# facebookresearch/FRL-Distributed-ML-Scaffold

Measured on NVIDIA H100. Metric: samples/sec (whole box) on synthetic 2-task Problem, higher is better.
Workload: dtype bf16

## Files before the change

### frl-distributed-ml-scaffold_b200/_native.py

```python
import ctypes as C
import os
import subprocess
from typing import Optional, Sequence

import torch

_HERE = os.path.dirname(os.path.abspath(__file__))
CSRC_DIR = os.path.join(_HERE, "csrc")
LIB_PATH = os.path.join(CSRC_DIR, "libfrl_b200.so")

F32, BF16, U8, I64 = 0, 1, 2, 3
LOSS_MSE, LOSS_CE, LOSS_CE_PROB = 0, 1, 2
FP8_E4M3, FP8_E5M2 = 0, 1
FP8_DTYPE = {FP8_E4M3: torch.float8_e4m3fn, FP8_E5M2: torch.float8_e5m2}
MAX_TASKS = 8

_DTYPE_CODE = {torch.float32: F32, torch.bfloat16: BF16, torch.uint8: U8, torch.bool: U8,
               torch.int64: I64}


class NativeLibraryError(RuntimeError):
    pass


# ... 3 lines not shown
        ("ignore_index", C.c_int32),
        ("out", C.c_void_p), ("tgt", C.c_void_p), ("mask", C.c_void_p), ("dout", C.c_void_p),
        ("rows", C.c_int64), ("cols", C.c_int64), ("mask_inner", C.c_int64),
        ("weight", C.c_float), ("label_smoothing", C.c_float),
    ]


class GradSeg(C.Structure):
    _fields_ = [("g", C.c_void_p), ("arena_off", C.c_int64), ("numel", C.c_int64),
                ("g_dtype", C.c_int32), ("_pad", C.c_int32)]


_vp, _i, _i64, _f, _d = C.c_void_p, C.c_int, C.c_int64, C.c_float, C.c_double
SIGNATURES = {
    "frl_abi_version": (_i, []),
    "frl_last_error": (C.c_char_p, []),
    "frl_launch_count": (C.c_uint64, []),
    "frl_launch_count_reset": (None, []),
    "frl_device_sm_count": (_i, []),
    "frl_device_arch": (_i, []),
    "frl_sgd_momentum": (_i, [_vp, _vp, _vp, _vp, _i64, _d, _d, _d, _d, _d, _vp, _vp, _i, _i, _vp]),
    "frl_adam": (_i, [_vp, _vp, _vp, _vp, _vp, _vp, _i64, _d, _d, _d, _d, _d, _i64, _d, _vp, _vp, _i, _vp]),
    "frl_rmsprop": (_i, [_vp, _vp, _vp, _vp, _vp, _i64, _d, _d, _d, _d, _d, _d, _vp, _vp, _i, _vp]),
    "frl_mt_tile_elems": (_i64, []),
    "frl_flatten_grads": (_i, [_vp, _vp, _vp, _i64, _vp, _i, _d, _vp]),
    "frl_sgd_momentum_mt": (_i, [_vp, _vp, _vp, _vp, _vp, _vp, _i64, _d, _d, _d, _d, _d, _vp, _vp, _i, _vp]),
    "frl_adam_mt": (_i, [_vp, _vp, _vp, _vp, _vp, _vp, _vp, _vp, _i64, _d, _d, _d, _d, _d, _i64, _d, _vp, _vp, _vp]),
    "frl_rmsprop_mt": (_i, [_vp, _vp, _vp, _vp, _vp, _vp, _vp, _i64, _d, _d, _d, _d, _d, _d, _vp, _vp, _vp]),
    "frl_layerwise_scratch_bytes": (_i64, [_i64, _i64]),
    "frl_lars_mt": (_i, [_vp, _vp, _vp, _vp, _vp, _vp, _i64, _i64, _vp, _vp, _vp, _d, _d, _d, _d, _vp, _vp, _i, _vp]),
    "frl_lamb_mt": (_i, [_vp, _vp, _vp, _vp, _vp, _vp, _vp, _i64, _i64, _vp, _vp, _vp, _d, _d, _d, _d, _d, _i64,
                         _d, _vp, _vp, _vp]),
    "frl_grad_accumulate_mt": (_i, [_vp, _vp, _vp, _vp, _i64, _d, _i, _vp, _vp]),
    "frl_weight_ema": (_i, [_vp, _vp, _i64, _d, _vp]),
    "frl_reduce_scratch_bytes": (_i64, []),
    "frl_grad_sumsq_clip": (_i, [_vp, _i64, _i, _f, _f, _vp, _vp, _vp]),
    "frl_criteria_scratch_bytes": (_i64, [_i]),
    "frl_criteria_forward": (_i, [C.POINTER(TaskDesc), _i, _vp, _vp, _vp, _vp, _vp, _vp, _vp]),
    "frl_criteria_backward": (_i, [C.POINTER(TaskDesc), _i, _vp, _vp, _vp, _vp]),
    "frl_preproc_affine": (_i, [_vp, _i, _vp, _i, _i64, _i64, _i64, _vp, _vp, _vp]),
    "frl_cast_scale": (_i, [_vp, _i, _vp, _i, _i64, _f, _vp]),
    "frl_augment_images": (_i, [_vp, _i64, _i, _i, _i, _vp, C.c_uint64, _i, _i, _d, _d, _d, _d, _d, _i, _i,
                                _vp, _vp, _vp, _i, _i, _i, _vp, _vp]),
    "frl_augment_mix_images": (_i, [_vp, _i64, _i, _i, _i, _vp, C.c_uint64, _i, _i, _d, _d, _d, _d, _d, _i, _i,
                                    _vp, _vp, _vp, _i, _i, _i, _vp, _i, _f, _i, _i, _i, _i, _vp]),
    "frl_mix_targets": (_i, [_vp, _i, _i64, _i64, _i, _f, _vp, _vp]),
# ... 89 lines not shown

def sgd_momentum(p, g, buf, p_lp, n, *, lr, mu, dampening, wd, grad_scale=1.0,
                 grad_scale_dev=None, first_step=False, dyn=None) -> None:
    _check(lib().frl_sgd_momentum(_ptr(p), _ptr(g), _ptr(buf), _ptr(p_lp), n, lr, mu, dampening,
                                  wd, grad_scale, _ptr(grad_scale_dev), _ptr(dyn), int(first_step),
                                  dtype_code(g.dtype), _stream()), "frl_sgd_momentum")


def adam(p, g, m, v, vmax, p_lp, n, *, lr, beta1, beta2, eps, wd, step, grad_scale=1.0,
         grad_scale_dev=None, dyn=None) -> None:
    _check(lib().frl_adam(_ptr(p), _ptr(g), _ptr(m), _ptr(v), _ptr(vmax), _ptr(p_lp), n, lr,
                          beta1, beta2, eps, wd, step, grad_scale, _ptr(grad_scale_dev), _ptr(dyn),
                          dtype_code(g.dtype), _stream()), "frl_adam")


def rmsprop(p, g, sq, buf, p_lp, n, *, lr, alpha, eps, wd, mu, grad_scale=1.0,
            grad_scale_dev=None, dyn=None) -> None:
    _check(lib().frl_rmsprop(_ptr(p), _ptr(g), _ptr(sq), _ptr(buf), _ptr(p_lp), n, lr, alpha,
                             eps, wd, mu, grad_scale, _ptr(grad_scale_dev), _ptr(dyn),
                             dtype_code(g.dtype), _stream()), "frl_rmsprop")



def mt_tile_elems() -> int:
    return int(lib().frl_mt_tile_elems())


def flatten_grads(table, arena_grad, *, scale: float = 1.0) -> None:
    _check(lib().frl_flatten_grads(table.segs_dev_ptr, table.prefix_dev_ptr, table.tile_seg_dev_ptr, table.n_tiles,
                                   _ptr(arena_grad), dtype_code(arena_grad.dtype), scale, _stream()),
           "frl_flatten_grads")


def sgd_momentum_mt(p, buf, p_lp, table, *, lr, mu, dampening, wd, grad_scale=1.0, grad_scale_dev=None,
                    first_step=False, dyn=None) -> None:
    _check(lib().frl_sgd_momentum_mt(_ptr(p), _ptr(buf), _ptr(p_lp), table.segs_dev_ptr, table.prefix_dev_ptr,
                                     table.tile_seg_dev_ptr, table.n_tiles, lr, mu, dampening, wd, grad_scale,
                                     _ptr(grad_scale_dev), _ptr(dyn), int(first_step), _stream()),
           "frl_sgd_momentum_mt")


def adam_mt(p, m, v, vmax, p_lp, table, *, lr, beta1, beta2, eps, wd, step, grad_scale=1.0,
            grad_scale_dev=None, dyn=None) -> None:
    _check(lib().frl_adam_mt(_ptr(p), _ptr(m), _ptr(v), _ptr(vmax), _ptr(p_lp), table.segs_dev_ptr,
                             table.prefix_dev_ptr, table.tile_seg_dev_ptr, table.n_tiles, lr, beta1, beta2, eps, wd,
                             step, grad_scale, _ptr(grad_scale_dev), _ptr(dyn), _stream()), "frl_adam_mt")
# ... 342 lines not shown
```

### frl-distributed-ml-scaffold_b200/arena_linear.py

```python
import os
import types
from collections import Counter
from typing import List, Optional

import torch
import torch.nn as nn
import torch.nn.functional as F

from . import _native
from .types import Precision

KERNELS = _native

FP8_MULTIPLE = 16


def fp8_site_qualifies(uses_lp: bool, in_features: int, out_features: int) -> bool:
    return bool(uses_lp) and in_features % FP8_MULTIPLE == 0 and out_features % FP8_MULTIPLE == 0


def fp8_call_qualifies(x: torch.Tensor) -> bool:
    if x.dim() == 0 or x.shape[-1] == 0 or x.dtype not in (torch.bfloat16, torch.float32):
        return False
    m = x.numel() // x.shape[-1]
# ... 255 lines not shown

class LinearSite:
    __slots__ = ("module", "wslot", "bslot", "pipeline", "relu", "wstate", "bstate", "multihead", "fp8")

    def __init__(self, module, wslot, bslot, pipeline):
        self.module = module
        self.wslot = wslot
        self.bslot = bslot
        self.pipeline = pipeline
        self.relu = None
        self.multihead = None
        self.fp8 = False
        states = pipeline.slot_states
        self.wstate = states.setdefault(wslot.index, SlotState())
        self.bstate = states.setdefault(bslot.index, SlotState()) if bslot is not None else None

    def weight_grad(self, pipe, gemms) -> None:
        gw = pipe.arena.grad_view(self.wslot)
        st = self.wstate
        if not st.first_touch(pipe.step_id):
            gemms.dw_add(gw)
            return
        rows = pipe.row_split(self.wslot)
        if (rows and rows % gemms.row_multiple == 0 and st.fwd_gen == pipe.forward_gen
                and st.fwd_count == 1):
            gemms.dw(gemms.dzt[:rows], out=gw[:rows])
            pipe.rows_ready(self.wslot, rows)
            gemms.dw(gemms.dzt[rows:], out=gw[rows:])
        else:
            gemms.dw(gemms.dzt, out=gw)

    def count_forward(self) -> None:
        pipe = self.pipeline
        if pipe is not None and self.module.training and torch.is_grad_enabled():
            gen = pipe.forward_gen
            self.wstate.count_forward(gen)
            if self.bstate is not None:
                self.bstate.count_forward(gen)

    def backward_done(self, pipe) -> None:
        step, gen = pipe.step_id, pipe.forward_gen
        if self.wstate.backward_complete(step, gen):
            pipe.mark_ready(self.wslot)
        else:
            pipe.defer_ready(self.wslot)
        if self.bstate is not None:
            if self.bstate.backward_complete(step, gen):
                pipe.mark_ready(self.bslot)
            else:
                pipe.defer_ready(self.bslot)

# ... 114 lines not shown
```

### frl-distributed-ml-scaffold_b200/fused_optim.py

```python
from typing import Any, Dict, List, Optional, Tuple

import torch

from . import _native
from .arena import ParamArena
from .types import LayerAdaptation, OptAlgorithm, OptimOpts

KERNELS = _native


class FusedArenaOptimizer(torch.optim.Optimizer):

    STATE_NAMES: Tuple[str, ...] = ()

    @property
    def needs_whole_tensors(self) -> bool:
        return False

    def __init__(self, arena: ParamArena, defaults: Dict[str, Any]) -> None:
        self.arena = arena
        params = arena.all_params
        if not params:
            raise ValueError("optimizer got an empty parameter list")
        super().__init__(params, defaults)
# ... 167 lines not shown
            elif entry:
                steps = max(steps, 1)
        self._steps = steps


class FusedSGD(FusedArenaOptimizer):
    STATE_NAMES = (("momentum_buffer", "momentum_buffer"),)

    def __init__(self, arena, lr, momentum=0.0, dampening=0.0, weight_decay=0.0):
        super().__init__(arena, dict(lr=lr, momentum=momentum, dampening=dampening,
                                     weight_decay=weight_decay, nesterov=False, maximize=False,
                                     foreach=None, differentiable=False, fused=None))

    def _launch(self, lo, hi, grad_scale, coef):
        h = self.hyper
        p, g, lp = self._slices(lo, hi)
        mu = float(h["momentum"])
        buf = self._state("momentum_buffer")[lo:hi] if mu != 0.0 else None
        KERNELS.sgd_momentum(p, g, buf, lp, hi - lo, lr=float(h["lr"]), mu=mu,
                             dampening=float(h["dampening"]), wd=float(h["weight_decay"]),
                             grad_scale=grad_scale, grad_scale_dev=coef,
                             first_step=(self._steps == 0), dyn=self._dyn)

    def _launch_mt(self, table, grad_scale):
        h = self.hyper
        mu = float(h["momentum"])
        KERNELS.sgd_momentum_mt(self.arena.master, self._state("momentum_buffer") if mu != 0.0 else None,
                                self.arena.lp, table, lr=float(h["lr"]), mu=mu,
                                dampening=float(h["dampening"]), wd=float(h["weight_decay"]),
                                grad_scale=grad_scale, first_step=(self._steps == 0), dyn=self._dyn)

    def _launch_nvls(self, lo, hi, grad_scale):
        h = self.hyper
        mu = float(h["momentum"])
        mc_g, mc_out = self._nvls_ptrs(lo)
        buf = self._state("momentum_buffer")[lo:hi] if mu != 0.0 else None
        KERNELS.nvls_sgd(self.arena.master[lo:hi], buf, mc_g, mc_out, hi - lo, self.nvls,
                         lr=float(h["lr"]), mu=mu, dampening=float(h["dampening"]),
                         wd=float(h["weight_decay"]), grad_scale=grad_scale,
                         first_step=(self._steps == 0),
                         g_dtype=KERNELS.dtype_code(self.arena.grad.dtype), dyn=self._dyn)


class FusedAdam(FusedArenaOptimizer):
    STATE_NAMES = (("exp_avg", "exp_avg"), ("exp_avg_sq", "exp_avg_sq"),
                   ("max_exp_avg_sq", "max_exp_avg_sq"))
# ... 214 lines not shown
```

### frl-distributed-ml-scaffold_b200/grad_sync.py

```python
import os
from typing import Callable, Dict, List, NamedTuple, Optional, Tuple

import torch
import torch.distributed as dist
import torch.nn as nn

from . import _native
from .arena import ParamArena
from .fused_optim import FusedArenaOptimizer

KERNELS = _native


class MicroBatch(NamedTuple):
    first: bool
    closes: bool
    rows: int
    weight: float
    group_rows: int


def accumulation_plan(n_batches: int, k: int, batch_size: int = 1,
                      n_samples: Optional[int] = None) -> List[MicroBatch]:
    if n_batches <= 0:
        return []
    last = batch_size if n_samples is None else n_samples - (n_batches - 1) * batch_size
    if not 0 < last <= batch_size:
        raise ValueError("%r samples do not make %d batches of %d" % (n_samples, n_batches, batch_size))
    rows = [batch_size] * (n_batches - 1) + [last]
    plan: List[MicroBatch] = []
    for lo in range(0, n_batches, k):
        group = rows[lo:lo + k]
# ... 119 lines not shown
        self._deferred = {}
        self.mt_enabled = (self.on_cuda and hasattr(KERNELS, "flatten_grads")
                           and os.environ.get("FRL_B200_MT_GRADS", "1") != "0")
        self._ext: Dict[int, torch.Tensor] = {}
        self.tables = _TableSet(arena)
        self._keep_ext = False
        self.record_update_events = False
        self.update_events: List[Tuple[torch.cuda.Event, torch.cuda.Event, int, int]] = []
        self.accumulate_events: List[Tuple[torch.cuda.Event, torch.cuda.Event]] = []

        self.acc: Optional[torch.Tensor] = None
        if self.accumulation > 1:
            self.acc = torch.zeros(arena.numel, dtype=torch.float32, device=arena.device)
            self._acc_dyn = torch.ones(2, dtype=torch.float32, device=arena.device)
            self._acc_dyn_host = torch.zeros(self._ACC_RING, 2, dtype=torch.float32, pin_memory=self.on_cuda)
            self._acc_dyn_slot = 0
            self._acc_dyn_last: Optional[Tuple[float, float]] = (1.0, 1.0)
        self._acc_first = True
        self._acc_closes = True
        self._acc_weight = 1.0
        self._acc_scale = self.grad_scale
        self._acc_seen = set()
        self.last_ready: frozenset = frozenset()

    _ACC_RING = 16

    @property
    def accumulator_bytes(self) -> int:
        return 0 if self.acc is None else self.acc.numel() * 4

    def set_microbatch(self, *, first: bool, closes: bool, weight: float = 1.0,
                       group_scale: float = 1.0) -> None:
        if self.acc is None:
            return
        self._acc_first, self._acc_closes = bool(first), bool(closes)
        self._acc_weight = float(weight)
        self._acc_scale = float(group_scale) / self.world
        if first:
            self._acc_seen.clear()
        vals = (self._acc_weight, 1.0 if first else 0.0)
        if vals != self._acc_dyn_last:
            if self.on_cuda:
                row = self._acc_dyn_host[self._acc_dyn_slot % self._ACC_RING]
                self._acc_dyn_slot += 1
                row[0], row[1] = vals
                self._acc_dyn.copy_(row, non_blocking=True)
            else:
                self._acc_dyn.copy_(torch.tensor(vals, dtype=torch.float32))
            self._acc_dyn_last = vals

    def begin_step(self) -> None:
        self._ready = 0
        self._ready_ids.clear()
        self._deferred.clear()
        for b in self.buckets:
            b.pending = len(b.slots)
            b.work = None
            b.launched = False
        self.optimizer.begin_step()
        self.step_id += 1
        self._step_open = True

    @property
    def step_open(self) -> bool:
        return self._step_open

    def _make_hook(self, slot) -> Callable[[nn.Parameter], None]:
        from .multi_tensor import grad_usable_in_place

        def hook(param: nn.Parameter) -> None:
            g = param.grad
            if g is not None:
                dst = self.arena.grad_view(slot)
                if g.data_ptr() != dst.data_ptr():
                    if self.mt_enabled and self._step_open and grad_usable_in_place(g, slot):
                        self._ext[slot.index] = g
                    else:
                        dst.copy_(g)
                param.grad = None
            self.mark_ready(slot)
        return hook

# ... 33 lines not shown
    def mark_ready(self, slot) -> None:
        if not self._step_open or id(slot.param) in self._ready_ids:
            return
        self._ready_ids.add(id(slot.param))
        self._ready += 1
        for b in self._buckets_of[id(slot.param)]:
            if b.launched:
                continue
            b.pending -= 1
            if b.pending == 0 and (self.distributed or self.eager) and self.acc is None:
                self._launch_bucket(b)

    def row_split(self, slot) -> int:
        return self._row_split.get(slot.index, 0)

    def rows_ready(self, slot, rows: int) -> None:
        if not self._step_open:
            return
        done = slot.offset + rows * slot.shape[1]
        for b in self._buckets_of[id(slot.param)]:
            if not b.launched and b.hi <= done and b.pending == 1:
                b.pending = 0
                self._launch_bucket(b)

    def defer_ready(self, slot) -> None:
        self._deferred[slot.index] = slot

    def _launch_bucket(self, b: _Bucket) -> None:
        if self.on_cuda:
            cur = torch.cuda.current_stream()
            self.side_stream.wait_stream(cur)
            torch.cuda.set_stream(self.side_stream)
        try:
            if self._ext:
                self._flatten_stragglers(b.slots, id(b), side=self.on_cuda)
            fused = self.nvls is not None and not b.replicated
            if self.distributed and not fused:
                b.work = dist.all_reduce(self.arena.grad[b.lo:b.hi], op=dist.ReduceOp.SUM,
                                         group=self.pg, async_op=True)
                if self.eager:
                    b.work.wait()
            if self.eager:
                tap = self._tap()
                if fused:
                    nv = self.nvls
                    grid = nv.max_blocks
# ... 42 lines not shown
            self._accumulate_microbatch(keep_refs=defer_tail)
        else:
            if self.distributed and not self.eager:
                cur = torch.cuda.current_stream() if self.on_cuda else None
                if cur is not None:
                    torch.cuda.set_stream(self.side_stream)
                for b in self.buckets:
                    b.work.wait()
                if cur is not None:
                    torch.cuda.set_stream(cur)
            if self.on_cuda and (self.distributed or self.eager):
                torch.cuda.current_stream().wait_stream(self.side_stream)
            if partial:
                self._end_update([s for s in self.arena.slots if id(s.param) in self._ready_ids],
                                 ema=not defer_tail)
                return
        if not defer_tail:
            self.run_tail()

    @property
    def has_tail(self) -> bool:
        return not self.eager

    def run_tail(self, grad_refs=None, tables=None, ready=None) -> None:
        if self.acc is not None:
            if ready is not None:
                self._acc_seen |= ready
            if self._acc_closes:
                self._end_update(acc=True)
            return
        if grad_refs is not None:
            mine = (self._ext, self.tables)
            self._ext, self.tables, self._keep_ext = grad_refs, tables, True
        try:
            if self.has_tail:
                self._end_update()
            else:
                self.optimizer.end_step()
                if self.ema is not None:
                    self.ema.update()
        finally:
            if grad_refs is not None:
                (self._ext, self.tables), self._keep_ext = mine, False

    def _end_update(self, present=None, acc: bool = False, ema: bool = True) -> None:
        slots, n = self.arena.slots, self.arena.numel
        if acc:
            grads, scale = self.acc, self._acc_scale
            if self.distributed:
                for b in self.buckets:
                    dist.all_reduce(grads[b.lo:b.hi], op=dist.ReduceOp.SUM, group=self.pg)
            else:
                present = [s for s in slots if s.index in self._acc_seen]
        else:
            grads, scale = self.arena.grad, self.grad_scale
        have = {s.index for s in (slots if present is None else present)}
        every = len(have) == len(slots)
        window = self._tap() if acc else None
        coef = None
        if not acc and (self.clip_norm > 0.0 or not every):
            self._flatten_stragglers(slots, "all", side=False)
        if self.clip_norm > 0.0:
            if not acc:
                for s in slots:
                    if s.index not in have and s.is_model:
                        grads[s.offset:s.end].zero_()
            n_model = self.arena.model_end
            KERNELS.grad_sumsq_clip(grads[:n_model], n_model, pre_scale=scale, max_norm=self.clip_norm,
                                    out3=self.clip_out, scratch=self.clip_scratch)
            coef = self.clip_out[2:3]
        if self.whole_tensors or (not acc and self._ext and coef is None and not self.distributed):
            table = self._table("acc" if acc else "grads", [s for s in slots if s.index in have], acc=acc)
            tap = None if acc else self._tap()
            self.optimizer.apply_table(table, grad_scale=scale, clip_coef_dev=coef)
            self._tap_end(tap, self.update_events, 0, n)
        else:
            done = [(b.lo, b.hi) for b in self.buckets if b.launched and self.eager]
            runs = [(0, n)] if every else self._runs(
                lambda s: s.index in have and not any(a <= s.offset < z for a, z in done))
            for lo, hi in runs:
                tap = None if acc else self._tap()
                self.optimizer.apply_range(lo, hi, grad_scale=scale, clip_coef_dev=coef,
                                           grad_src=grads if acc else None)
                self._tap_end(tap, self.update_events, lo, hi)
        self._tap_end(window, self.update_events, 0, n)
        if not self._keep_ext:
            self._ext.clear()
        self.optimizer.end_step()
        if ema and self.ema is not None:
            self.ema.update()

    def _runs(self, keep) -> List[Tuple[int, int]]:
        runs: List[Tuple[int, int]] = []
        run_lo = prev_end = None
        for s in self.arena.slots:
            if not keep(s):
                if run_lo is not None:
                    runs.append((run_lo, prev_end))
                    run_lo = None
                continue
            if run_lo is None:
# ... 92 lines not shown
```

### frl-distributed-ml-scaffold_b200/graph_step.py

```python
from typing import Dict, List, Optional, Sequence, Tuple

import gc
import logging

import torch

from . import _native

logger = logging.getLogger(__name__)

REPLAYED_LAUNCHES = 0


def _signature(data: Sequence[torch.Tensor], target) -> Tuple:
    sig = [(tuple(t.shape), t.dtype) for t in data]
    for head in target:
        sig.append(tuple((tuple(t.shape), t.dtype) for t in head))
    return tuple(sig)


class GraphedTrainStep:
    WARMUP_STEPS = 2

    def __init__(self, worker) -> None:
# ... 40 lines not shown
        for t in data:
            cast = bf16 and t.dtype == torch.float32
            self.static_in.append(torch.empty_like(t, dtype=torch.bfloat16 if cast else t.dtype))
            self.cast_in.append(cast)
        self.static_tgt = [tuple(torch.empty_like(t) for t in head) for head in target]
        self._fill(data, target)

        w.optimizer.enable_dynamic_scalars()
        w.criterion.set_step_sink(None, None)
        gc.collect()
        torch.cuda.synchronize()
        self.graph = torch.cuda.CUDAGraph()
        launches_before = _native.launch_count()
        with torch.cuda.graph(self.graph, capture_error_mode="thread_local"):
            if w.buffers is not None:
                w.buffers.sync()
            output = w.model(self.static_in)
            total, sub = w.criterion(output, self.static_tgt)
            w.pipeline.begin_step()
            total.backward()
            w.pipeline.finish_step(defer_tail=True)
        self.grad_refs, self.tables = w.pipeline.detach_grad_refs()
        self.ready = w.pipeline.last_ready
        w.pipeline.step_id -= 1
        self.frl_kernels = _native.launch_count() - launches_before
        self.output = [o.detach() for o in output]
        self.names = list(sub.keys())
        self._total, self._sub = total.detach(), {k: v.detach() for k, v in sub.items()}
        base = getattr(total, "_base", None)
        self._loss_vec = base.detach() if (base is not None and base.dim() == 1
                                           and base.numel() == 1 + len(self.names)
                                           and base.dtype == torch.float32) else None

    def _fill(self, data, target) -> None:
        for dst, src, cast in zip(self.static_in, data, self.cast_in):
            if cast:
                _native.cast_scale(src.contiguous(), dst, 1.0)
            else:
                dst.copy_(src, non_blocking=True)
        for dhead, shead in zip(self.static_tgt, target):
            for d, s in zip(dhead, shead):
                d.copy_(s, non_blocking=True)

    def run(self, data, target, sink_row: Optional[torch.Tensor]):
        w = self.worker
        self._fill(data, target)
        w.optimizer.refresh_dynamic_scalars()
        self.graph.replay()
        global REPLAYED_LAUNCHES
        REPLAYED_LAUNCHES += self.frl_kernels
        w.pipeline.step_id += 1
        w.pipeline.run_tail(self.grad_refs, self.tables, self.ready)
        if sink_row is not None:
            row = self._loss_vec
            if row is None:
                row = torch.stack([self._total.float()] + [self._sub[k].float() for k in self.names])
            sink_row.copy_(row, non_blocking=True)
            w.criterion._sink_written = True
        return self.output, self._total, self._sub
```

### frl-distributed-ml-scaffold_b200/solver.py

```python
import io
import json
import logging
import math
import multiprocessing
import os
import pickle
import traceback
from collections import defaultdict
from contextlib import ExitStack
from multiprocessing.connection import Connection, wait as wait_pipes
from typing import IO, Any, DefaultDict, Dict, Iterator, List, NamedTuple, Optional, Sequence

import numpy as np
import torch
import torch.nn as nn

from .arena import ParamArena
from .criteria import BaseParallelCriterion
from .ema import EMA_STATE_KEY
from .fused_optim import check_layer_adaptation, create_fused_optimizer, is_adapted
from .grad_sync import BufferBroadcaster, GradBucketPipeline
from .lr_scheduler import DropEpochsScheduler, WarmupMultiStepLR
from .problem import Problem
from .solver_worker import (FractionalPerformanceSummary, SerializableSampleSummary,
# ... 341 lines not shown
        if distributed:
            pipeline.broadcast_parameters(src=0)
            buffers = BufferBroadcaster(model, world_size=args.world_size)
            buffers.sync()
        worker = SolverWorker(model, criterion, optimizer, device=device, run_opts=run_opts,
                              cache=args.cache, local_rank=args.local_rank,
                              node_idx=args.node_idx, node_count=args.node_count,
                              pipeline=pipeline, buffers=buffers, precision=args.precision,
                              serialize_state=(args.local_rank == 0),
                              graph_step=(args.graph_step if args.graph_step is not None
                                          else os.environ.get("FRL_B200_CUDA_GRAPH", "0") == "1"),
                              ema=ema)
        worker.save_every = args.save_every
        if args.rank == 0:
            logger.info(
                "frl_b200 step: precision %s | step issue %s | gradient exchange %s | update %s | "
                "Linear layers with arena-born gradients %d (%d fused with their ReLU, %d in FP8) | "
                "other gradients %s | layer adaptation %s | gradient accumulation %s | weight EMA %s",
                args.precision.value,
                "CUDA-graph replay after 2 eager steps" if worker.graphed is not None else "eager launches",
                ("fused NVLS kernel per bucket (K7), %d buckets" % len(pipeline.buckets)) if pipeline.nvls is not None
                else ("ncclAllReduce in place + K2 per bucket, %d buckets" % len(pipeline.buckets)) if distributed
                else "none (1 GPU)",
                "per bucket on the side stream" if pipeline.eager else "one tail launch",
                len(pipeline.linear_sites), sum(s.relu is not None for s in pipeline.linear_sites),
                sum(s.fp8 for s in pipeline.linear_sites),
                "read in place through segment tables (K2-mt / one flatten launch per bucket)"
                if pipeline.mt_enabled else "copied into the arena per tensor",
                "none" if args.layer_adaptation == LayerAdaptation.NONE else
                "%s, %d of %d tensors adapted (K2-lw)" % (args.layer_adaptation.value,
                                                          sum(is_adapted(s) for s in arena.slots), len(arena.slots)),
                "none" if accum == 1 else
                "%d microbatches per update (K10, fp32 accumulator %.1f MiB)" % (
                    accum, pipeline.accumulator_bytes / 2 ** 20),
                "none" if ema is None else
                "decay %r, one K11 launch per update (%.1f MiB), held-out splits evaluated with it" % (
                    ema_decay, ema.nbytes / 2 ** 20))
        scheduler = create_lr_scheduler(run_opts, worker.optimizer,
                                        checkpoint.epoch if checkpoint else -1)
        return worker, scheduler, checkpoint

    @classmethod
    def _run_solver_worker(cls, args: SolverWorkerArgs) -> Iterator[FractionalPerformanceSummary]:
        worker, scheduler, checkpoint = cls.build_worker(args)
        run_opts = args.run_opts
        if run_opts.mode == Mode.TRAIN:
            yield from worker.train(args.problem,
# ... 255 lines not shown
```

### include/frl_b200.h

```cpp
#ifndef FRL_B200_H
#define FRL_B200_H

#include <stdint.h>

#ifdef __cplusplus
extern "C" {
#endif

#define FRL_ABI_VERSION 1

enum { FRL_F32 = 0, FRL_BF16 = 1, FRL_U8 = 2, FRL_I64 = 3 };
enum { FRL_E_ARG = -1, FRL_E_ALIGN = -2, FRL_E_DTYPE = -3, FRL_E_TOO_MANY = -4 };

int          frl_abi_version(void);
const char*  frl_last_error(void);
uint64_t     frl_launch_count(void);
void         frl_launch_count_reset(void);
int          frl_device_sm_count(void);
int          frl_device_arch(void);


int frl_sgd_momentum(float* p, const void* g, float* buf, void* p_lp, int64_t n,
                     double lr, double mu, double dampening, double wd,
                     double grad_scale, const float* grad_scale_dev, const float* dyn,
                     int first_step, int g_dtype, void* stream);

int frl_adam(float* p, const void* g, float* m, float* v, float* vmax, void* p_lp, int64_t n,
             double lr, double beta1, double beta2, double eps, double wd, int64_t step,
             double grad_scale, const float* grad_scale_dev, const float* dyn, int g_dtype,
             void* stream);

int frl_rmsprop(float* p, const void* g, float* sq, float* buf, void* p_lp, int64_t n,
                double lr, double alpha, double eps, double wd, double mu,
                double grad_scale, const float* grad_scale_dev, const float* dyn, int g_dtype,
             void* stream);

typedef struct frl_grad_seg {
    const void* g;
    int64_t     arena_off;
    int64_t     numel;
    int32_t     g_dtype;
    int32_t     _pad;
} frl_grad_seg;

int64_t frl_mt_tile_elems(void);

int frl_flatten_grads(const frl_grad_seg* segs_dev, const int64_t* tile_prefix_dev,
                      const int32_t* tile_seg_dev, int64_t n_tiles, void* arena_grad, int dst_dtype,
                      double scale, void* stream);

int frl_sgd_momentum_mt(float* p, float* buf, void* p_lp, const frl_grad_seg* segs_dev,
                        const int64_t* tile_prefix_dev, const int32_t* tile_seg_dev, int64_t n_tiles,
                        double lr, double mu, double dampening, double wd, double grad_scale,
                        const float* grad_scale_dev, const float* dyn, int first_step, void* stream);

int frl_adam_mt(float* p, float* m, float* v, float* vmax, void* p_lp, const frl_grad_seg* segs_dev,
                const int64_t* tile_prefix_dev, const int32_t* tile_seg_dev, int64_t n_tiles, double lr, double beta1,
                double beta2, double eps, double wd, int64_t step, double grad_scale,
// ... 140 lines not shown
```

Baseline: 1.931 million.

## Fuse SGD update into a custom WGMMA weight-gradient GEMM epilogue

Result: faster. 2.081 million, median of 6 (+7.8%).

```diff
diff --git a/frl-distributed-ml-scaffold_b200/_native.py b/frl-distributed-ml-scaffold_b200/_native.py
--- a/frl-distributed-ml-scaffold_b200/_native.py
+++ b/frl-distributed-ml-scaffold_b200/_native.py
@@ -49,6 +49,9 @@
     "frl_sgd_momentum": (_i, [_vp, _vp, _vp, _vp, _i64, _d, _d, _d, _d, _d, _vp, _vp, _i, _i, _vp]),
     "frl_adam": (_i, [_vp, _vp, _vp, _vp, _vp, _vp, _i64, _d, _d, _d, _d, _d, _i64, _d, _vp, _vp, _i, _vp]),
     "frl_rmsprop": (_i, [_vp, _vp, _vp, _vp, _vp, _i64, _d, _d, _d, _d, _d, _d, _vp, _vp, _i, _vp]),
+    "frl_dw_gemm": (_i, [_vp, _i64, _vp, _i64, _i64, _i64, _i64, _vp, _vp]),
+    "frl_dw_gemm_sgd": (_i, [_vp, _i64, _vp, _i64, _i64, _i64, _i64, _vp, _vp, _vp, _vp, _d, _d, _d, _d, _d,
+                             _vp, _i, _vp]),
     "frl_mt_tile_elems": (_i64, []),
     "frl_flatten_grads": (_i, [_vp, _vp, _vp, _i64, _vp, _i, _d, _vp]),
     "frl_sgd_momentum_mt": (_i, [_vp, _vp, _vp, _vp, _vp, _vp, _i64, _d, _d, _d, _d, _d, _vp, _vp, _i, _vp]),
@@ -184,6 +187,31 @@
 
 
 
+DW_TILE = (128, 256, 64)
+
+
+def dw_gemm_fits(dz, x, gw) -> bool:
+    tm, tn, tk = DW_TILE
+    return (dz.dim() == 2 and x.dim() == 2 and dz.dtype == x.dtype == gw.dtype == torch.bfloat16
+            and dz.stride(1) == 1 and x.stride(1) == 1 and dz.stride(0) % 8 == 0 and x.stride(0) % 8 == 0
+            and dz.data_ptr() % 16 == 0 and x.data_ptr() % 16 == 0 and gw.data_ptr() % 16 == 0
+            and gw.is_contiguous() and dz.shape[0] == x.shape[0] and tuple(gw.shape) == (dz.shape[1], x.shape[1])
+            and dz.shape[1] % tm == 0 and x.shape[1] % tn == 0 and dz.shape[0] % tk == 0 and dz.shape[0] > 0)
+
+
+def dw_gemm(dz, x, gw) -> None:
+    _check(lib().frl_dw_gemm(_ptr(dz), dz.stride(0), _ptr(x), x.stride(0), dz.shape[0], dz.shape[1], x.shape[1],
+                             _ptr(gw), _stream()), "frl_dw_gemm")
+
+
+def dw_gemm_sgd(dz, x, gw, p, buf, p_lp, *, lr, mu, dampening, wd, grad_scale=1.0, first_step=False,
+                dyn=None) -> None:
+    _check(lib().frl_dw_gemm_sgd(_ptr(dz), dz.stride(0), _ptr(x), x.stride(0), dz.shape[0], dz.shape[1],
+                                 x.shape[1], _ptr(gw), _ptr(p), _ptr(buf), _ptr(p_lp), lr, mu, dampening, wd,
+                                 grad_scale, _ptr(dyn), int(first_step), _stream()), "frl_dw_gemm_sgd")
+
+
+
 def mt_tile_elems() -> int:
     return int(lib().frl_mt_tile_elems())
 
diff --git a/frl-distributed-ml-scaffold_b200/arena_linear.py b/frl-distributed-ml-scaffold_b200/arena_linear.py
--- a/frl-distributed-ml-scaffold_b200/arena_linear.py
+++ b/frl-distributed-ml-scaffold_b200/arena_linear.py
@@ -301,11 +301,14 @@
             gemms.dw_add(gw)
             return
         rows = pipe.row_split(self.wslot)
-        if (rows and rows % gemms.row_multiple == 0 and st.fwd_gen == pipe.forward_gen
-                and st.fwd_count == 1):
+        only_use = st.fwd_gen == pipe.forward_gen and st.fwd_count == 1
+        if rows and rows % gemms.row_multiple == 0 and only_use:
             gemms.dw(gemms.dzt[:rows], out=gw[:rows])
             pipe.rows_ready(self.wslot, rows)
             gemms.dw(gemms.dzt[rows:], out=gw[rows:])
+        elif (pipe.fused_dw_update and only_use and not rows and type(gemms) is _DenseGemms
+              and self.wslot.uses_lp and _native.dw_gemm_fits(gemms.dz, gemms.x2, gw)):
+            pipe.update_in_dw_gemm(self.wslot, gemms.dz, gemms.x2, gw)
         else:
             gemms.dw(gemms.dzt, out=gw)
 
diff --git a/frl-distributed-ml-scaffold_b200/csrc/dw_update.cu b/frl-distributed-ml-scaffold_b200/csrc/dw_update.cu
--- /dev/null
+++ b/frl-distributed-ml-scaffold_b200/csrc/dw_update.cu
@@ -0,0 +1,375 @@
+#include <cuda.h>
+
+#include "frl_common.cuh"
+#include "optim_rules.cuh"
+
+namespace frl {
+namespace dw {
+
+constexpr int kBM = 128, kBN = 256, kBK = 32, kStages = 6;
+constexpr int kThreads = 384;
+constexpr int kEpiThreads = 96;
+constexpr int kTailWarps = 11;
+constexpr int kAtomBytes = 64 * kBK * 2;
+constexpr int kABytes = 2 * kAtomBytes;
+constexpr int kBBytes = 4 * kAtomBytes;
+constexpr int kStageBytes = kABytes + kBBytes;
+constexpr int kStagingBytes = kBM * kBN * 2;
+constexpr int kSmemBytes = 1024 + kStages * kStageBytes + kStagingBytes + 256;
+static_assert(kBK % 16 == 0 && kBK <= 256, "k-block must be a multiple of the WGMMA K");
+static_assert(kSmemBytes <= 227 * 1024, "shared memory plan exceeds one CTA per SM");
+
+__device__ __forceinline__ uint32_t smem_u32(const void* p) {
+    return static_cast<uint32_t>(__cvta_generic_to_shared(p));
+}
+__device__ __forceinline__ void mbar_init(uint64_t* bar, uint32_t count) {
+    asm volatile("mbarrier.init.shared::cta.b64 [%0], %1;" :: "r"(smem_u32(bar)), "r"(count));
+}
+__device__ __forceinline__ void mbar_expect_tx(uint64_t* bar, uint32_t bytes) {
+    asm volatile("mbarrier.arrive.expect_tx.shared::cta.b64 _, [%0], %1;"
+                 :: "r"(smem_u32(bar)), "r"(bytes) : "memory");
+}
+__device__ __forceinline__ void mbar_arrive(uint64_t* bar) {
+    asm volatile("mbarrier.arrive.shared::cta.b64 _, [%0];" :: "r"(smem_u32(bar)) : "memory");
+}
+__device__ __forceinline__ void mbar_wait(uint64_t* bar, uint32_t parity) {
+    asm volatile(
+        "{\n"
+        ".reg .pred p;\n"
+        "WAIT_%=:\n"
+        "mbarrier.try_wait.parity.shared::cta.b64 p, [%0], %1;\n"
+        "@!p bra WAIT_%=;\n"
+        "}\n" :: "r"(smem_u32(bar)), "r"(parity) : "memory");
+}
+__device__ __forceinline__ void tma_load_2d(void* dst, const CUtensorMap* map, int c0, int c1, uint64_t* bar) {
+    asm volatile(
+        "cp.async.bulk.tensor.2d.shared::cluster.global.mbarrier::complete_tx::bytes [%0], [%1, {%2, %3}], [%4];"
+        :: "r"(smem_u32(dst)), "l"(map), "r"(c0), "r"(c1), "r"(smem_u32(bar)) : "memory");
+}
+
+__device__ __forceinline__ uint64_t desc_mn_sw128(uint32_t addr, uint32_t lbo, uint32_t sbo) {
+    return static_cast<uint64_t>((addr & 0x3FFFF) >> 4) | (static_cast<uint64_t>(lbo >> 4) << 16) |
+           (static_cast<uint64_t>(sbo >> 4) << 32) | (1ull << 62);
+}
+
+__device__ __forceinline__ void fence_acc(float* d) {
+#pragma unroll
+    for (int i = 0; i < 128; ++i) asm volatile("" : "+f"(d[i]) :: "memory");
+}
+
+__device__ __forceinline__ void wgmma_m64n256k16(float* d, uint64_t da, uint64_t db, int accumulate) {
+    asm volatile(
+        "{\n"
+        ".reg .pred p;\n"
+        "setp.ne.b32 p, %130, 0;\n"
+        "wgmma.mma_async.sync.aligned.m64n256k16.f32.bf16.bf16 {"
+        "%0, %1, %2, %3, %4, %5, %6, %7, %8, %9, %10, %11, %12, %13, %14, %15,"
+        "%16, %17, %18, %19, %20, %21, %22, %23, %24, %25, %26, %27, %28, %29, %30, %31,"
+        "%32, %33, %34, %35, %36, %37, %38, %39, %40, %41, %42, %43, %44, %45, %46, %47,"
+        "%48, %49, %50, %51, %52, %53, %54, %55, %56, %57, %58, %59, %60, %61, %62, %63,"
+        "%64, %65, %66, %67, %68, %69, %70, %71, %72, %73, %74, %75, %76, %77, %78, %79,"
+        "%80, %81, %82, %83, %84, %85, %86, %87, %88, %89, %90, %91, %92, %93, %94, %95,"
+        "%96, %97, %98, %99, %100, %101, %102, %103, %104, %105, %106, %107, %108, %109, %110, %111,"
+        "%112, %113, %114, %115, %116, %117, %118, %119, %120, %121, %122, %123, %124, %125, %126, %127"
+        "}, %128, %129, p, 1, 1, 1, 1;\n"
+        "}\n"
+        : "+f"(d[0]), "+f"(d[1]), "+f"(d[2]), "+f"(d[3]), "+f"(d[4]), "+f"(d[5]), "+f"(d[6]), "+f"(d[7]),
+          "+f"(d[8]), "+f"(d[9]), "+f"(d[10]), "+f"(d[11]), "+f"(d[12]), "+f"(d[13]), "+f"(d[14]), "+f"(d[15]),
+          "+f"(d[16]), "+f"(d[17]), "+f"(d[18]), "+f"(d[19]), "+f"(d[20]), "+f"(d[21]), "+f"(d[22]), "+f"(d[23]),
+          "+f"(d[24]), "+f"(d[25]), "+f"(d[26]), "+f"(d[27]), "+f"(d[28]), "+f"(d[29]), "+f"(d[30]), "+f"(d[31]),
+          "+f"(d[32]), "+f"(d[33]), "+f"(d[34]), "+f"(d[35]), "+f"(d[36]), "+f"(d[37]), "+f"(d[38]), "+f"(d[39]),
+          "+f"(d[40]), "+f"(d[41]), "+f"(d[42]), "+f"(d[43]), "+f"(d[44]), "+f"(d[45]), "+f"(d[46]), "+f"(d[47]),
+          "+f"(d[48]), "+f"(d[49]), "+f"(d[50]), "+f"(d[51]), "+f"(d[52]), "+f"(d[53]), "+f"(d[54]), "+f"(d[55]),
+          "+f"(d[56]), "+f"(d[57]), "+f"(d[58]), "+f"(d[59]), "+f"(d[60]), "+f"(d[61]), "+f"(d[62]), "+f"(d[63]),
+          "+f"(d[64]), "+f"(d[65]), "+f"(d[66]), "+f"(d[67]), "+f"(d[68]), "+f"(d[69]), "+f"(d[70]), "+f"(d[71]),
+          "+f"(d[72]), "+f"(d[73]), "+f"(d[74]), "+f"(d[75]), "+f"(d[76]), "+f"(d[77]), "+f"(d[78]), "+f"(d[79]),
+          "+f"(d[80]), "+f"(d[81]), "+f"(d[82]), "+f"(d[83]), "+f"(d[84]), "+f"(d[85]), "+f"(d[86]), "+f"(d[87]),
+          "+f"(d[88]), "+f"(d[89]), "+f"(d[90]), "+f"(d[91]), "+f"(d[92]), "+f"(d[93]), "+f"(d[94]), "+f"(d[95]),
+          "+f"(d[96]), "+f"(d[97]), "+f"(d[98]), "+f"(d[99]), "+f"(d[100]), "+f"(d[101]), "+f"(d[102]), "+f"(d[103]),
+          "+f"(d[104]), "+f"(d[105]), "+f"(d[106]), "+f"(d[107]), "+f"(d[108]), "+f"(d[109]), "+f"(d[110]), "+f"(d[111]),
+          "+f"(d[112]), "+f"(d[113]), "+f"(d[114]), "+f"(d[115]), "+f"(d[116]), "+f"(d[117]), "+f"(d[118]), "+f"(d[119]),
+          "+f"(d[120]), "+f"(d[121]), "+f"(d[122]), "+f"(d[123]), "+f"(d[124]), "+f"(d[125]), "+f"(d[126]), "+f"(d[127])
+        : "l"(da), "l"(db), "r"(accumulate));
+}
+
+__device__ __forceinline__ void tile_origin(int tile, int tiles_m, int tiles_n, int& m0, int& n0) {
+    const int g = (tiles_m % 16 == 0) ? 16 : tiles_m;
+    const int per_group = g * tiles_n;
+    const int in = tile % per_group;
+    m0 = ((tile / per_group) * g + in % g) * kBM;
+    n0 = (in / g) * kBN;
+}
+
+__device__ __forceinline__ uint32_t staging_off(int row, int col) {
+    return static_cast<uint32_t>(row * (kBN * 2) + ((((col >> 3) ^ (row & 7)) << 4) | ((col & 7) << 1)));
+}
+
+struct Update {
+    float* master;
+    float* mom;
+    __nv_bfloat16* lp;
+    SgdRule rule;
+    float gscale;
+    const float* dyn;
+};
+
+__device__ __forceinline__ void sgd4(const SgdRule& r, f32x4& p, f32x4& m, float g0, float g1, float g2,
+                                     float g3, float gs) {
+    float dummy0 = 0.f, dummy1 = 0.f;
+    r(p.x, g0 * gs, m.x, dummy0, dummy1);
+    r(p.y, g1 * gs, m.y, dummy0, dummy1);
+    r(p.z, g2 * gs, m.z, dummy0, dummy1);
+    r(p.w, g3 * gs, m.w, dummy0, dummy1);
+}
+
+template <bool UPDATE>
+__device__ __forceinline__ void epilogue_rows(const uint8_t* staging, __nv_bfloat16* gw, int64_t ld,
+                                              int64_t m0, int64_t n0, const Update& u, int e, int n, int lane) {
+    constexpr int kRowsAtOnce = 4;
+    for (int r0 = e; r0 < kBM; r0 += n * kRowsAtOnce) {
+        f32x4 p[kRowsAtOnce][2], m[kRowsAtOnce][2];
+        bf16x4 g[kRowsAtOnce][2];
+#pragma unroll
+        for (int j = 0; j < kRowsAtOnce; ++j) {
+            const int r = r0 + n * j;
+            if (r >= kBM) break;
+            const int64_t row = (m0 + r) * ld + n0;
+#pragma unroll
+            for (int h = 0; h < 2; ++h) {
+                const int col = h * 128 + 4 * lane;
+                g[j][h] = *reinterpret_cast<const bf16x4*>(staging + staging_off(r, col));
+                if (UPDATE) {
+                    p[j][h] = ld_stream(reinterpret_cast<const f32x4*>(u.master + row + col));
+                    if (u.mom) m[j][h] = ld_stream(reinterpret_cast<const f32x4*>(u.mom + row + col));
+                }
+            }
+        }
+#pragma unroll
+        for (int j = 0; j < kRowsAtOnce; ++j) {
+            const int r = r0 + n * j;
+            if (r >= kBM) break;
+            const int64_t row = (m0 + r) * ld + n0;
+#pragma unroll
+            for (int h = 0; h < 2; ++h) {
+                const int col = h * 128 + 4 * lane;
+                st_stream(reinterpret_cast<bf16x4*>(gw + row + col), g[j][h]);
+                if (UPDATE) {
+                    f32x4 q = p[j][h], s = u.mom ? m[j][h] : f32x4{0.f, 0.f, 0.f, 0.f};
+                    sgd4(u.rule, q, s, bf16lo(g[j][h].a), bf16hi(g[j][h].a), bf16lo(g[j][h].b),
+                         bf16hi(g[j][h].b), u.gscale);
+                    st_stream(reinterpret_cast<f32x4*>(u.master + row + col), q);
+                    if (u.mom) st_stream(reinterpret_cast<f32x4*>(u.mom + row + col), s);
+                    if (u.lp)
+                        st_stream(reinterpret_cast<bf16x4*>(u.lp + row + col),
+                                  bf16x4{pack_bf16(q.x, q.y), pack_bf16(q.z, q.w)});
+                }
+            }
+        }
+    }
+}
+
+template <bool UPDATE>
+__global__ void __launch_bounds__(kThreads, 1)
+dw_gemm_kernel(const __grid_constant__ CUtensorMap tm_dz, const __grid_constant__ CUtensorMap tm_x,
+               int M, int N, int K, __nv_bfloat16* __restrict__ gw, Update u) {
+    extern __shared__ uint8_t smem_raw[];
+    uint8_t* smem = reinterpret_cast<uint8_t*>((reinterpret_cast<uintptr_t>(smem_raw) + 1023) & ~uintptr_t(1023));
+    uint8_t* staging = smem + kStages * kStageBytes;
+    uint64_t* full = reinterpret_cast<uint64_t*>(staging + kStagingBytes);
+    uint64_t* empty = full + kStages;
+    uint64_t* epi_full = empty + kStages;
+    uint64_t* epi_empty = epi_full + 1;
+
+    const int warp = threadIdx.x >> 5, lane = threadIdx.x & 31;
+    if (threadIdx.x == 0) {
+        for (int s = 0; s < kStages; ++s) {
+            mbar_init(&full[s], 1);
+            mbar_init(&empty[s], 8);
+        }
+        mbar_init(epi_full, 256);
+        mbar_init(epi_empty, kEpiThreads);
+        asm volatile("fence.mbarrier_init.release.cluster;" ::: "memory");
+        asm volatile("prefetch.tensormap [%0];" :: "l"(&tm_dz) : "memory");
+        asm volatile("prefetch.tensormap [%0];" :: "l"(&tm_x) : "memory");
+    }
+    __syncthreads();
+
+    const int tiles_m = M / kBM, tiles_n = N / kBN, n_tiles = tiles_m * tiles_n, n_kb = K / kBK;
+
+    if (warp == 0) {
+        if (lane == 0) {
+            int stage = 0;
+            uint32_t phase = 0;
+            for (int tile = blockIdx.x; tile < n_tiles; tile += gridDim.x) {
+                int m0, n0;
+                tile_origin(tile, tiles_m, tiles_n, m0, n0);
+                for (int kb = 0; kb < n_kb; ++kb) {
+                    mbar_wait(&empty[stage], phase ^ 1);
+                    mbar_expect_tx(&full[stage], kStageBytes);
+                    uint8_t* a = smem + stage * kStageBytes;
+                    uint8_t* b = a + kABytes;
+                    const int k0 = kb * kBK;
+                    tma_load_2d(a, &tm_dz, m0, k0, &full[stage]);
+                    tma_load_2d(a + kAtomBytes, &tm_dz, m0 + 64, k0, &full[stage]);
+#pragma unroll
+                    for (int j = 0; j < 4; ++j) tma_load_2d(b + j * kAtomBytes, &tm_x, n0 + 64 * j, k0, &full[stage]);
+                    if (++stage == kStages) { stage = 0; phase ^= 1; }
+                }
+            }
+        }
+        return;
+    }
+    if (warp < 4) {
+        Update upd = u;
+        if (UPDATE && upd.dyn) upd.rule.patch(upd.dyn);
+        int it = 0;
+        for (int tile = blockIdx.x; tile < n_tiles; tile += gridDim.x, ++it) {
+            int m0, n0;
+            tile_origin(tile, tiles_m, tiles_n, m0, n0);
+            const bool last = tile + static_cast<int>(gridDim.x) >= n_tiles;
+            mbar_wait(epi_full, it & 1);
+            epilogue_rows<UPDATE>(staging, gw, N, m0, n0, upd, warp - 1, last ? kTailWarps : 3, lane);
+            mbar_arrive(epi_empty);
+        }
+        return;
+    }
+
+    const int cw = (threadIdx.x >> 7) - 1;
+    const int t = threadIdx.x & 127, wi = t >> 5;
+    const uint32_t smem_base = smem_u32(smem);
+    float d[128];
+    int stage = 0;
+    uint32_t phase = 0;
+    int it = 0;
+    for (int tile = blockIdx.x; tile < n_tiles; tile += gridDim.x, ++it) {
+        int prev = -1;
+        for (int kb = 0; kb < n_kb; ++kb) {
+            mbar_wait(&full[stage], phase);
+            const uint32_t a = smem_base + stage * kStageBytes + cw * kAtomBytes;
+            const uint32_t b = smem_base + stage * kStageBytes + kABytes;
+            fence_acc(d);
+            asm volatile("wgmma.fence.sync.aligned;" ::: "memory");
+#pragma unroll
+            for (int kk = 0; kk < kBK / 16; ++kk)
+                wgmma_m64n256k16(d, desc_mn_sw128(a + kk * 2048, kAtomBytes, 1024),
+                                 desc_mn_sw128(b + kk * 2048, kAtomBytes, 1024), (kb | kk) != 0);
+            asm volatile("wgmma.commit_group.sync.aligned;" ::: "memory");
+            asm volatile("wgmma.wait_group.sync.aligned 1;" ::: "memory");
+            fence_acc(d);
+            if (prev >= 0 && lane == 0) mbar_arrive(&empty[prev]);
+            prev = stage;
+            if (++stage == kStages) { stage = 0; phase ^= 1; }
+        }
+        asm volatile("wgmma.wait_group.sync.aligned 0;" ::: "memory");
+        fence_acc(d);
+        if (lane == 0) mbar_arrive(&empty[prev]);
+
+        mbar_wait(epi_empty, (it & 1) ^ 1);
+        const int row = 64 * cw + 16 * wi + (lane >> 2);
+        uint8_t* base = staging + row * (kBN * 2) + 4 * (lane & 3);
+#pragma unroll
+        for (int c7 = 0; c7 < 8; ++c7) {
+            uint8_t* p = base + ((c7 ^ (row & 7)) << 4);
+#pragma unroll
+            for (int cg = 0; cg < 4; ++cg) {
+                const int c = 8 * cg + c7;
+                *reinterpret_cast<uint32_t*>(p + 128 * cg) = pack_bf16(d[4 * c], d[4 * c + 1]);
+                *reinterpret_cast<uint32_t*>(p + 128 * cg + 8 * kBN * 2) = pack_bf16(d[4 * c + 2], d[4 * c + 3]);
+            }
+        }
+        mbar_arrive(epi_full);
+    }
+    if (it > 0) {
+        const int tile = blockIdx.x + (it - 1) * gridDim.x;
+        Update upd = u;
+        if (UPDATE && upd.dyn) upd.rule.patch(upd.dyn);
+        mbar_wait(epi_full, (it - 1) & 1);
+        int m0, n0;
+        tile_origin(tile, tiles_m, tiles_n, m0, n0);
+        epilogue_rows<UPDATE>(staging, gw, N, m0, n0, upd,
+                              3 + (warp - 4), kTailWarps, lane);
+    }
+}
+
+typedef CUresult (*EncodeTiledFn)(CUtensorMap*, CUtensorMapDataType, cuuint32_t, void*, const cuuint64_t*,
+                                  const cuuint64_t*, const cuuint32_t*, const cuuint32_t*, CUtensorMapInterleave,
+                                  CUtensorMapSwizzle, CUtensorMapL2promotion, CUtensorMapFloatOOBfill);
+
+static EncodeTiledFn encode_fn() {
+    static EncodeTiledFn fn = nullptr;
+    if (!fn) {
+        void* p = nullptr;
+        cudaDriverEntryPointQueryResult q;
+        if (cudaGetDriverEntryPoint("cuTensorMapEncodeTiled", &p, cudaEnableDefault, &q) == cudaSuccess &&
+            q == cudaDriverEntryPointSuccess)
+            fn = reinterpret_cast<EncodeTiledFn>(p);
+    }
+    return fn;
+}
+
+static bool encode(CUtensorMap* map, const void* base, int64_t rows, int64_t cols, int64_t ld) {
+    EncodeTiledFn fn = encode_fn();
+    if (!fn) return false;
+    const cuuint64_t dims[2] = {static_cast<cuuint64_t>(cols), static_cast<cuuint64_t>(rows)};
+    const cuuint64_t strides[1] = {static_cast<cuuint64_t>(ld) * 2};
+    const cuuint32_t box[2] = {64, static_cast<cuuint32_t>(kBK)};
+    const cuuint32_t estr[2] = {1, 1};
+    return fn(map, CU_TENSOR_MAP_DATA_TYPE_BFLOAT16, 2, const_cast<void*>(base), dims, strides, box, estr,
+              CU_TENSOR_MAP_INTERLEAVE_NONE, CU_TENSOR_MAP_SWIZZLE_128B, CU_TENSOR_MAP_L2_PROMOTION_L2_256B,
+              CU_TENSOR_MAP_FLOAT_OOB_FILL_NONE) == CUDA_SUCCESS;
+}
+
+template <bool UPDATE>
+static int launch(const void* dz, int64_t ld_dz, const void* x, int64_t ld_x, int64_t rows, int64_t out,
+                  int64_t in, void* gw, const Update& u, cudaStream_t st, const char* name) {
+    FRL_REQUIRE(dz && x && gw, FRL_E_ARG, "%s: null operand", name);
+    FRL_REQUIRE(out % kBM == 0 && in % kBN == 0 && rows % kBK == 0 && rows > 0, FRL_E_ARG,
+                "%s: shape [%lld x %lld] over %lld rows is not a multiple of the %dx%dx%d tile", name,
+                static_cast<long long>(out), static_cast<long long>(in), static_cast<long long>(rows),
+                kBM, kBN, kBK);
+    FRL_REQUIRE(out <= INT32_MAX && in <= INT32_MAX && rows <= INT32_MAX, FRL_E_ARG, "%s: shape too large", name);
+    FRL_REQUIRE(ld_dz >= out && ld_x >= in && ld_dz % 8 == 0 && ld_x % 8 == 0, FRL_E_ARG,
+                "%s: leading dimensions must cover the rows and be multiples of 8", name);
+    FRL_REQUIRE(aligned16(dz) && aligned16(x) && aligned16(gw) && aligned16(u.master) && aligned16(u.mom) &&
+                aligned16(u.lp), FRL_E_ALIGN, "%s: arrays must be 16-byte aligned", name);
+    CUtensorMap tm_dz, tm_x;
+    FRL_REQUIRE(encode(&tm_dz, dz, rows, out, ld_dz) && encode(&tm_x, x, rows, in, ld_x), FRL_E_ARG,
+                "%s: cuTensorMapEncodeTiled failed", name);
+    static bool attr_set = false;
+    if (!attr_set) {
+        const cudaError_t e = cudaFuncSetAttribute(dw_gemm_kernel<UPDATE>,
+                                                   cudaFuncAttributeMaxDynamicSharedMemorySize, kSmemBytes);
+        FRL_REQUIRE(e == cudaSuccess, static_cast<int>(e), "%s: smem attribute: %s", name, cudaGetErrorString(e));
+        attr_set = true;
+    }
+    const int n_tiles = static_cast<int>((out / kBM) * (in / kBN));
+    const int grid = n_tiles < sm_count() ? n_tiles : sm_count();
+    dw_gemm_kernel<UPDATE><<<grid, kThreads, kSmemBytes, st>>>(
+        tm_dz, tm_x, static_cast<int>(out), static_cast<int>(in), static_cast<int>(rows),
+        static_cast<__nv_bfloat16*>(gw), u);
+    return after_launch(name);
+}
+
+}
+}
+
+using namespace frl;
+
+extern "C" int frl_dw_gemm(const void* dz, int64_t ld_dz, const void* x, int64_t ld_x, int64_t rows,
+                           int64_t out, int64_t in, void* gw, void* stream) {
+    dw::Update u{};
+    return dw::launch<false>(dz, ld_dz, x, ld_x, rows, out, in, gw, u, static_cast<cudaStream_t>(stream),
+                             "frl_dw_gemm");
+}
+
+extern "C" int frl_dw_gemm_sgd(const void* dz, int64_t ld_dz, const void* x, int64_t ld_x, int64_t rows,
+                               int64_t out, int64_t in, void* gw, float* p, float* buf, void* p_lp,
+                               double lr, double mu, double dampening, double wd, double grad_scale,
+                               const float* dyn, int first_step, void* stream) {
+    FRL_REQUIRE(p, FRL_E_ARG, "frl_dw_gemm_sgd: null master");
+    FRL_REQUIRE(mu == 0.0 || buf != nullptr, FRL_E_ARG, "frl_dw_gemm_sgd: momentum needs buf");
+    dw::Update u{p, mu != 0.0 ? buf : nullptr, static_cast<__nv_bfloat16*>(p_lp),
+                 make_sgd_rule(lr, mu, dampening, wd, first_step), static_cast<float>(grad_scale), dyn};
+    return dw::launch<true>(dz, ld_dz, x, ld_x, rows, out, in, gw, u, static_cast<cudaStream_t>(stream),
+                            "frl_dw_gemm_sgd");
+}
diff --git a/frl-distributed-ml-scaffold_b200/fused_optim.py b/frl-distributed-ml-scaffold_b200/fused_optim.py
--- a/frl-distributed-ml-scaffold_b200/fused_optim.py
+++ b/frl-distributed-ml-scaffold_b200/fused_optim.py
@@ -213,6 +213,16 @@
                              grad_scale=grad_scale, grad_scale_dev=coef,
                              first_step=(self._steps == 0), dyn=self._dyn)
 
+    def update_in_dw_gemm(self, slot, dz, x, gw, *, grad_scale: float = 1.0) -> None:
+        h = self.hyper
+        a = self.arena
+        mu = float(h["momentum"])
+        buf = self._state("momentum_buffer")[slot.offset:slot.end] if mu != 0.0 else None
+        KERNELS.dw_gemm_sgd(dz, x, gw, a.master[slot.offset:slot.end], buf, a.lp[slot.offset:slot.end],
+                            lr=float(h["lr"]), mu=mu, dampening=float(h["dampening"]),
+                            wd=float(h["weight_decay"]), grad_scale=grad_scale,
+                            first_step=(self._steps == 0), dyn=self._dyn)
+
     def _launch_mt(self, table, grad_scale):
         h = self.hyper
         mu = float(h["momentum"])
diff --git a/frl-distributed-ml-scaffold_b200/grad_sync.py b/frl-distributed-ml-scaffold_b200/grad_sync.py
--- a/frl-distributed-ml-scaffold_b200/grad_sync.py
+++ b/frl-distributed-ml-scaffold_b200/grad_sync.py
@@ -7,7 +7,8 @@
 
 from . import _native
 from .arena import ParamArena
-from .fused_optim import FusedArenaOptimizer
+from .fused_optim import FusedArenaOptimizer, FusedSGD
+from .types import Precision
 
 KERNELS = _native
 
@@ -173,6 +174,12 @@
         self._acc_scale = self.grad_scale
         self._acc_seen = set()
         self.last_ready: frozenset = frozenset()
+        self.fused_dw_update = (
+            not self.distributed and not self.eager and self.clip_norm == 0.0 and self.accumulation == 1
+            and type(optimizer) is FusedSGD and arena.precision is Precision.BF16
+            and hasattr(KERNELS, "dw_gemm_sgd") and (self.on_cuda or KERNELS is not _native)
+            and os.environ.get("FRL_B200_FUSED_DW_UPDATE", "1") != "0")
+        self.dw_updated: set = set()
 
     _ACC_RING = 16
 
@@ -209,6 +216,7 @@
             b.work = None
             b.launched = False
         self.optimizer.begin_step()
+        self.dw_updated = set()
         self.step_id += 1
         self._step_open = True
 
@@ -288,6 +296,10 @@
             if not b.launched and b.hi <= done and b.pending == 1:
                 b.pending = 0
                 self._launch_bucket(b)
+
+    def update_in_dw_gemm(self, slot, dz, x, gw) -> None:
+        self.optimizer.update_in_dw_gemm(slot, dz, x, gw, grad_scale=self.grad_scale)
+        self.dw_updated.add(slot.index)
 
     def defer_ready(self, slot) -> None:
         self._deferred[slot.index] = slot
@@ -376,7 +388,7 @@
     def has_tail(self) -> bool:
         return not self.eager
 
-    def run_tail(self, grad_refs=None, tables=None, ready=None) -> None:
+    def run_tail(self, grad_refs=None, tables=None, ready=None, dw_updated=None) -> None:
         if self.acc is not None:
             if ready is not None:
                 self._acc_seen |= ready
@@ -384,8 +396,10 @@
                 self._end_update(acc=True)
             return
         if grad_refs is not None:
-            mine = (self._ext, self.tables)
+            mine = (self._ext, self.tables, self.dw_updated)
             self._ext, self.tables, self._keep_ext = grad_refs, tables, True
+            if dw_updated is not None:
+                self.dw_updated = dw_updated
         try:
             if self.has_tail:
                 self._end_update()
@@ -395,7 +409,7 @@
                     self.ema.update()
         finally:
             if grad_refs is not None:
-                (self._ext, self.tables), self._keep_ext = mine, False
+                (self._ext, self.tables, self.dw_updated), self._keep_ext = mine, False
 
     def _end_update(self, present=None, acc: bool = False, ema: bool = True) -> None:
         slots, n = self.arena.slots, self.arena.numel
@@ -423,6 +437,8 @@
             KERNELS.grad_sumsq_clip(grads[:n_model], n_model, pre_scale=scale, max_norm=self.clip_norm,
                                     out3=self.clip_out, scratch=self.clip_scratch)
             coef = self.clip_out[2:3]
+        if not acc:
+            have -= self.dw_updated
         if self.whole_tensors or (not acc and self._ext and coef is None and not self.distributed):
             table = self._table("acc" if acc else "grads", [s for s in slots if s.index in have], acc=acc)
             tap = None if acc else self._tap()
@@ -430,7 +446,7 @@
             self._tap_end(tap, self.update_events, 0, n)
         else:
             done = [(b.lo, b.hi) for b in self.buckets if b.launched and self.eager]
-            runs = [(0, n)] if every else self._runs(
+            runs = [(0, n)] if len(have) == len(slots) else self._runs(
                 lambda s: s.index in have and not any(a <= s.offset < z for a, z in done))
             for lo, hi in runs:
                 tap = None if acc else self._tap()
diff --git a/frl-distributed-ml-scaffold_b200/graph_step.py b/frl-distributed-ml-scaffold_b200/graph_step.py
--- a/frl-distributed-ml-scaffold_b200/graph_step.py
+++ b/frl-distributed-ml-scaffold_b200/graph_step.py
@@ -86,6 +86,7 @@
             w.pipeline.finish_step(defer_tail=True)
         self.grad_refs, self.tables = w.pipeline.detach_grad_refs()
         self.ready = w.pipeline.last_ready
+        self.dw_updated = w.pipeline.dw_updated
         w.pipeline.step_id -= 1
         self.frl_kernels = _native.launch_count() - launches_before
         self.output = [o.detach() for o in output]
@@ -114,7 +115,7 @@
         global REPLAYED_LAUNCHES
         REPLAYED_LAUNCHES += self.frl_kernels
         w.pipeline.step_id += 1
-        w.pipeline.run_tail(self.grad_refs, self.tables, self.ready)
+        w.pipeline.run_tail(self.grad_refs, self.tables, self.ready, self.dw_updated)
         if sink_row is not None:
             row = self._loss_vec
             if row is None:
diff --git a/frl-distributed-ml-scaffold_b200/solver.py b/frl-distributed-ml-scaffold_b200/solver.py
--- a/frl-distributed-ml-scaffold_b200/solver.py
+++ b/frl-distributed-ml-scaffold_b200/solver.py
@@ -387,7 +387,9 @@
                 ("fused NVLS kernel per bucket (K7), %d buckets" % len(pipeline.buckets)) if pipeline.nvls is not None
                 else ("ncclAllReduce in place + K2 per bucket, %d buckets" % len(pipeline.buckets)) if distributed
                 else "none (1 GPU)",
-                "per bucket on the side stream" if pipeline.eager else "one tail launch",
+                "per bucket on the side stream" if pipeline.eager else
+                "in the dW GEMM's epilogue (K12) for trunk Linear weights that qualify, one tail launch for the rest"
+                if pipeline.fused_dw_update else "one tail launch",
                 len(pipeline.linear_sites), sum(s.relu is not None for s in pipeline.linear_sites),
                 sum(s.fp8 for s in pipeline.linear_sites),
                 "read in place through segment tables (K2-mt / one flatten launch per bucket)"
diff --git a/include/frl_b200.h b/include/frl_b200.h
--- a/include/frl_b200.h
+++ b/include/frl_b200.h
@@ -34,6 +34,13 @@
                 double lr, double alpha, double eps, double wd, double mu,
                 double grad_scale, const float* grad_scale_dev, const float* dyn, int g_dtype,
              void* stream);
+
+int frl_dw_gemm(const void* dz, int64_t ld_dz, const void* x, int64_t ld_x, int64_t rows,
+                int64_t out, int64_t in, void* gw, void* stream);
+int frl_dw_gemm_sgd(const void* dz, int64_t ld_dz, const void* x, int64_t ld_x, int64_t rows,
+                    int64_t out, int64_t in, void* gw, float* p, float* buf, void* p_lp,
+                    double lr, double mu, double dampening, double wd, double grad_scale,
+                    const float* dyn, int first_step, void* stream);
 
 typedef struct frl_grad_seg {
     const void* g;
```
